# jameschapman19/cca_zoo

Hardware: AMD Instinct MI355X
Metric: CCA fit()/sec at n=1e6 d=4096 k=64 (higher is better)
Workload: dtype f32

## Files before the change

### cca_zoo_amd/csrc/gemm64_big.hip

```cpp
#include <algorithm>
#include <cstdlib>

#include "hip_common.h"

namespace ccz {

typedef double v4f64 __attribute__((ext_vector_type(4)));
typedef double v2f64 __attribute__((ext_vector_type(2)));

constexpr int DT = 128;
constexpr int DK = 16;

constexpr int DS = DT + 2;

constexpr int HM = 64;

template <bool KMAJOR, int W>
struct StagerW {
  static constexpr int NI = W / 32;
  static constexpr int TPR = W / 2;
  static constexpr int RPP = 256 / TPR;
  v2f64 r[NI];
  __device__ __forceinline__ void load(const double* __restrict__ P, int64_t ld, int64_t m0, int64_t mlim, int64_t k0, int tid) {
    if (KMAJOR) {
// ... 22 lines not shown
#pragma unroll
      for (int i = 0; i < NI; ++i) *reinterpret_cast<v2f64*>(dst + (tid / TPR + RPP * i) * stride + 2 * (tid % TPR)) = r[i];
    } else {
      const int kq = tid & 7;
#pragma unroll
      for (int i = 0; i < NI; ++i) {
        const int m = (tid >> 3) + 32 * i;
        dst[(2 * kq) * stride + m] = r[i][0];
        dst[(2 * kq + 1) * stride + m] = r[i][1];
      }
    }
  }
};

template <bool TA, bool TB, int TM>
__global__ __launch_bounds__(256, 2) void k_gemm_f64_pipe(int64_t M, int64_t N, int64_t K, double alpha,
                                                          const double* __restrict__ A, int64_t lda,
                                                          const double* __restrict__ B, int64_t ldb, double beta,
                                                          double* __restrict__ C, int64_t ldc, int lower_only,
                                                          int64_t k_per_split) {
  constexpr int WN = TM == 128 ? 64 : 32;
  constexpr int NB = WN / 16;
  constexpr int SA = TM + 2;
  constexpr int BUF = DK * (SA + DS);
  constexpr int NSTG = TM / 32 + DT / 32;
  extern __shared__ __attribute__((aligned(16))) char smem_p[];
  double* lds = reinterpret_cast<double*>(smem_p);
  const int64_t m0 = int64_t(blockIdx.y) * TM, n0 = int64_t(blockIdx.x) * DT;
  if (lower_only && n0 > m0 + (TM - 1)) return;
  const int tid = threadIdx.x, lane = tid & 63, wave = tid >> 6;
  const int a_off = TM == 128 ? (wave >> 1) * 64 : 0;
  const int b_off = TM == 128 ? (wave & 1) * 64 : wave * 32;

  v4f64 acc[4][NB];
#pragma unroll
  for (int i = 0; i < 4; ++i)
#pragma unroll
    for (int j = 0; j < NB; ++j)
#pragma unroll
      for (int r = 0; r < 4; ++r) acc[i][j][r] = 0.0;

  StagerW<TA, TM> sa;
  StagerW<!TB, DT> sb;
  const bool split = gridDim.z > 1;
  const int64_t kz0 = int64_t(blockIdx.z) * k_per_split;
  const int64_t nkb = (min(K, kz0 + k_per_split) - kz0) / DK;
  if (nkb <= 0) return;

  auto rd = [&](const double* as, int kk, double (&a4)[4], double (&b4)[NB]) {
    const int krow = 4 * kk + (lane >> 4);
    const double* ap = as + krow * SA + a_off + 4 * (lane & 15);
    const v2f64 a01 = *reinterpret_cast<const v2f64*>(ap), a23 = *reinterpret_cast<const v2f64*>(ap + 2);
    a4[0] = a01[0]; a4[1] = a01[1]; a4[2] = a23[0]; a4[3] = a23[1];
    const double* bp = as + DK * SA + krow * DS + b_off + NB * (lane & 15);
    const v2f64 b01 = *reinterpret_cast<const v2f64*>(bp);
    b4[0] = b01[0]; b4[1] = b01[1];
    if constexpr (NB == 4) {
      const v2f64 b23 = *reinterpret_cast<const v2f64*>(bp + 2);
      b4[2] = b23[0]; b4[3] = b23[1];
    }
// ... 83 lines not shown
            v[q + 1] += beta * c01[1];
          }
        }
#pragma unroll
        for (int q = 0; q < NB; q += 2) *reinterpret_cast<v2f64*>(cp + q) = v2f64{v[q], v[q + 1]};
      } else {
#pragma unroll
        for (int tj = 0; tj < NB; ++tj)
          if (nb + tj < N) {
            double v = alpha * acc[ti][tj][r];
            if (beta != 0.0) v += beta * cp[tj];
            cp[tj] = v;
          }
      }
    }
}

bool gemm_f64_big_eligible(bool tA, bool tB, int64_t M, int64_t N, int64_t K, const double* A, int64_t lda,
                           const double* B, int64_t ldb, const double* C, int64_t ldc) {
  (void)tA; (void)tB;
  const int64_t min_tiles = env::once(env::GEMM_BIG_MIN_TILES), min_k = env::once(env::GEMM_BIG_MIN_K);
  if (K % DK != 0 || K < min_k) return false;
  if ((lda | ldb | ldc) & 1) return false;
  if ((reinterpret_cast<uintptr_t>(A) | reinterpret_cast<uintptr_t>(B) | reinterpret_cast<uintptr_t>(C)) & 15) return false;
  if ((M + DT - 1) / DT > 65535) return false;
  const int64_t tiles = (M + DT - 1) / DT * ((N + DT - 1) / DT);
  if (M >= 128 && N >= 128 && tiles >= min_tiles) return true;
  return false;
}

// ... 35 lines not shown
  } while (0)
#define CCZ_LAUNCH_PIPE_T(TM_)                              \
  do {                                                      \
    if (!tA && !tB) CCZ_LAUNCH_PIPE(false, false, TM_);     \
    else if (tA && !tB) CCZ_LAUNCH_PIPE(true, false, TM_);  \
    else if (!tA && tB) CCZ_LAUNCH_PIPE(false, true, TM_);  \
    else CCZ_LAUNCH_PIPE(true, true, TM_);                  \
  } while (0)
  if (use_half) CCZ_LAUNCH_PIPE_T(64);
  else CCZ_LAUNCH_PIPE_T(128);
#undef CCZ_LAUNCH_PIPE_T
#undef CCZ_LAUNCH_PIPE
  CCZ_LAUNCH_CHECK();
}

}
```

### cca_zoo_amd/csrc/gram.hip

```cpp
#include <algorithm>
#include <cstdio>
#include <cstdlib>
#include <cstring>
#include <thread>
#include <vector>

#include "hip_common.h"
#include "gram_map.h"

namespace ccz {

typedef float v16f32 __attribute__((ext_vector_type(16)));
typedef float v4f32 __attribute__((ext_vector_type(4)));
typedef double v4f64 __attribute__((ext_vector_type(4)));
typedef double v2f64 __attribute__((ext_vector_type(2)));

constexpr int BK = 16;

typedef const float __attribute__((address_space(1)))* gptr_f32;
typedef const double __attribute__((address_space(1)))* gptr_f64;

typedef unsigned int v4u32 __attribute__((ext_vector_type(4)));

constexpr int T32 = 256;
// ... 724 lines not shown
  const double sj = (t0 + t1) + (t2 + t3);
  sums[j] = sj;
  pilot[j] = float(sj / double(n));
}

__global__ void k_pilot_from_sums(const double* __restrict__ s, int64_t D, double inv_n, float* __restrict__ pilot) {
  const int64_t j = int64_t(blockIdx.x) * blockDim.x + threadIdx.x;
  if (j < D) pilot[j] = float(s[j] * inv_n);
}

__global__ void k_pilot_fixup(double* __restrict__ G, int64_t D, const double* __restrict__ s_launch, double n,
                              const float* __restrict__ pilot) {
  const int64_t i = blockIdx.y;
  const int64_t j = i + int64_t(blockIdx.x) * blockDim.x + threadIdx.x;
  if (j >= D) return;
  const double pi = double(pilot[i]), pj = double(pilot[j]);
  G[i * D + j] += pi * s_launch[j] + pj * s_launch[i] - n * pi * pj;
}

__global__ __launch_bounds__(256) void k_gram_reduce(const float* __restrict__ partial, const GramTile* __restrict__ tiles, int ntiles,
                                                     int64_t ksplit, double* __restrict__ G, int64_t ldg) {
  const int tile = blockIdx.y;
  const GramTile t = tiles[tile];
  const int e = blockIdx.x * 256 + threadIdx.x;
  const int i = e >> 8, j = e & 255;
  if (i >= t.wa || j >= t.wb) return;
  double acc = 0.0;
  const float* p = partial + int64_t(tile) * (T32 * T32) + e;
  for (int64_t c = 0; c < ksplit; ++c) acc += double(p[c * int64_t(ntiles) * (T32 * T32)]);
  G[(t.out_row + i) * ldg + t.out_col + j] += acc;
}

// ... 276 lines not shown
  hipStream_t st = stream(c);
  constexpr bool is32 = sizeof(T) == 4;
  const int ncu = std::max(1, im->props.multiProcessorCount);
  const int pilot_env = env::once(env::GRAM_PILOT);
  if (pilot_env == 0 || pilot_env == 1) pilot_mode = pilot_env == 1 ? 2 : 0;
  if (!is32) pilot_mode = 0;
  bool split = false;
  if (is32) {
    const char* e = env::once(env::K1_ROUTE);
    const int route_env = !e ? 0 : !strcmp(e, "fp32") ? int(CCZ_K1_FP32) : !strcmp(e, "bf16x2") ? int(CCZ_K1_BF16X2) : 0;
    const int route = c->k1_route != CCZ_K1_AUTO ? c->k1_route : route_env;
    split = (route == CCZ_K1_BF16X2 || (route == CCZ_K1_AUTO && gram_split_worthwhile(n, D))) && n_views <= 16;
    if (split) pilot_mode = 2;
  }
  c->last_route = !is32 ? CCZ_K1_FP64 : (split ? CCZ_K1_BF16X2 : CCZ_K1_FP32);
  if (pilot_mode == 2 && D > 65535) fail(CCZ_EUNSUP, "gram: pilot fix-up supports D <= 65535");
  TileTable tt;
  RowPlan rp;
  if (!split) {
    tt = build_tile_table<T>(c, views, n_views, tile_cache);
    rp = plan_rows<T>(c, views, n_views, n, tt.ntiles, tt.fast);
  }
  const double pilot_thr = env::once(env::GRAM_PILOT_RATIO);
  double* s_launch = s;
  double* sq = nullptr;
  PoolBuf<double> s_own;
  if (pilot_mode != 0) {
    s_own = PoolBuf<double>(c, D * (pilot_mode == 1 ? 2 : 1));
    s_launch = s_own;
    zero(c, s_launch, size_t(D) * 8 * (pilot_mode == 1 ? 2 : 1));
    if (pilot_mode == 1) sq = s_launch + D;
// ... 43 lines not shown
      const double mu = hs[j] / double(n), var = hs[D + j] / double(n) - mu * mu;
      if (!std::isfinite(mu) || !std::isfinite(var)) continue;
      const double sd = var > 0.0 ? std::sqrt(var) : 0.0;
      const double ratio = std::fabs(mu) <= pilot_thr * sd ? 0.0 : (sd > 0.0 ? std::fabs(mu) / sd : 1e300);
      if (ratio > worst) worst = ratio;
    }
    use_pilot = worst > pilot_thr;
    if (use_pilot && D > 65535) fail(CCZ_EUNSUP, "gram: pilot fix-up supports D <= 65535");
  }
  if (use_pilot && !split) {
    pilot = pilot_own = PoolBuf<float>(c, D);
    hipLaunchKernelGGL(k_pilot_from_sums, dim3((unsigned)((D + 255) / 256)), dim3(256), 0, st, s_launch, D, 1.0 / double(n), pilot);
  }

  if (time_it) CCZ_HIP(hipEventRecord(im->ev[0].get(), st));
  if (split) gram_split_f32(c, views, n_views, n, G, D, pilot, s_launch, time_it);
  else if (is32) launch_gram_f32(c, tt, rp, n, G, D, pilot);
  else launch_gram_f64(c, tt, rp, n, G, D);
  CCZ_LAUNCH_CHECK();
  if (time_it) CCZ_HIP(hipEventRecord(im->ev[1].get(), st));
  if (use_pilot) hipLaunchKernelGGL(k_pilot_fixup, dim3((unsigned)((D + 255) / 256), (unsigned)D), dim3(256), 0, st, G, D, s_launch, double(n), pilot);
  if (s_launch != s) hipLaunchKernelGGL(k_vec_add, dim3((unsigned)((D + 255) / 256)), dim3(256), 0, st, s, s_launch, D);
  CCZ_LAUNCH_CHECK();
  if (time_it) {
    CCZ_HIP(hipEventSynchronize(im->ev[1].get()));
    float g = 0.f, cs = 0.f;
    CCZ_HIP(hipEventElapsedTime(&g, im->ev[0].get(), im->ev[1].get()));
    CCZ_HIP(hipEventElapsedTime(&cs, im->ev[2].get(), im->ev[3].get()));
    c->last_gram_ms += g;
    c->last_colsum_ms += cs;
  }
  c->last_pilot = use_pilot ? 1 : 0;
  return use_pilot;
}

bool ensure_pipe(ccz_ctx* c, size_t bytes) {
// ... 289 lines not shown
```

### cca_zoo_amd/csrc/gram_split.hip

```cpp
#include <algorithm>
#include <vector>

#include "hip_common.h"
#include "gram_map.h"
#include "split_mma.h"

namespace ccz {

constexpr int SP_MAXV = 16;

struct SplitPanel {
  int32_t view;
  int32_t col0;
  int32_t width;
  int32_t gcol0;
};

struct SplitViews {
  const float* data[SP_MAXV];
  int64_t ld[SP_MAXV];
};

struct SplitTile {
  int32_t pa, pb;
// ... 156 lines not shown
    if (ti < ti0 || ti >= ti1) continue;
    float* prow = pt + (qr * 128 + ti * 32 + (lane & 31)) * SP_T + qc * 128 + 4 * (lane >> 5);
#pragma unroll
    for (int tj = 0; tj < 4; ++tj) {
      if (sym && tj < ti) continue;
#pragma unroll
      for (int g = 0; g < 4; ++g) {
        const sp_v4f32 v = {acc[ti][tj][4 * g], acc[ti][tj][4 * g + 1], acc[ti][tj][4 * g + 2], acc[ti][tj][4 * g + 3]};
        *reinterpret_cast<sp_v4f32*>(prow + tj * 32 + 8 * g) = v;
      }
    }
  }
}

__global__ __launch_bounds__(256) void k_split_reduce(const float* __restrict__ partial, const SplitTile* __restrict__ tiles, int ntiles,
                                                      int64_t ksplit, double* __restrict__ G, int64_t ldg, const double* __restrict__ msq) {
  const int tile = blockIdx.y;
  const SplitTile t = tiles[tile];
  const int e = (blockIdx.x * 256 + threadIdx.x) * 4;
  const int i = e >> 8, j = e & 255;
  if (i >= t.wa || j >= t.wb) return;
  double a0 = 0.0, a1 = 0.0, a2 = 0.0, a3 = 0.0;
  const float* p = partial + int64_t(tile) * (SP_T * SP_T) + e;
  const int64_t stride = int64_t(ntiles) * (SP_T * SP_T);
  for (int64_t c = 0; c < ksplit; ++c) {
    const sp_v4f32 v = __builtin_nontemporal_load(reinterpret_cast<const sp_v4f32*>(p + c * stride));
    a0 += double(v[0]); a1 += double(v[1]); a2 += double(v[2]); a3 += double(v[3]);
  }
  const double a[4] = {a0, a1, a2, a3};
  double* g = G + (int64_t(t.out_row) + i) * ldg + t.out_col + j;
#pragma unroll
  for (int q = 0; q < 4; ++q) {
    if (j + q >= t.wb) break;
    if (t.diag && j + q < i) continue;
    double v = a[q];
    if (t.diag && i == j + q) v += msq[t.out_row + i];
    g[q] += v;
  }
}

namespace {

std::vector<std::pair<int, int>> split_tile_order(int np) {
  std::vector<std::pair<int, int>> full, dg, rest;
  for (int I = 0; I < np; I += 4)
    for (int J = (I / 8) * 8; J < np; J += 8) {
      std::vector<std::pair<int, int>> blk;
      bool has_diag = false;
      for (int i = I; i < std::min(np, I + 4); ++i)
        for (int j = std::max(i, J); j < std::min(np, J + 8); ++j) { blk.emplace_back(i, j); has_diag = has_diag || i == j; }
      for (const auto& ij : blk) {
        if (blk.size() == 32 && !has_diag) full.push_back(ij);
// ... 177 lines not shown
  CCZ_LAUNCH_CHECK();
  out->tiles = tb.gtiles;
  out->ntiles = tb.ntiles;
  out->ksplit = rp.ksplit;
  c->last_pilot = 1;
  c->last_route = CCZ_K1_BF16X2;
  return true;
}

bool gram_split_worthwhile(int64_t n, int64_t D) {
  const double min_flop = env::live(env::SPLIT_MIN_FLOP);
  return n >= 32768 && D >= 256 && double(n) * double(D) * double(D + 1) >= min_flop;
}

void gram_split_f32(ccz_ctx* c, const ccz_view* views, int n_views, int64_t n, double* G, int64_t D, const float* pilot, double* colsum,
                    bool time_it) {
  Impl* im = impl(c);
  hipStream_t st = stream(c);
  if (n_views > SP_MAXV) fail(CCZ_EUNSUP, "gram (split route): more than %d views", SP_MAXV);
  if (D > 0x7fffffffLL - 256) fail(CCZ_EUNSUP, "gram (split route): stacked width too large");
  int64_t cols[SP_MAXV];
  for (int v = 0; v < n_views; ++v) cols[v] = views[v].cols;
  const SplitTables tb = split_tables(c, cols, n_views);
  SplitViews vws{};
  const bool aligned = split_views_arg(views, n_views, &vws);
  const int np = tb.np, ntiles = tb.ntiles;
  PoolBuf<double> msq(c, D);
  const int ncu = std::max(1, im->props.multiProcessorCount);
  const int64_t max_steps = std::max<int64_t>(1, env::live(env::SPLIT_ROWS) / SP_K);
  const int64_t unit = max_steps * SP_K;
  const double per_row = double(np) * SP_PSTEP / SP_K + double(ntiles) * (SP_T * SP_T * 4) / double(unit);
// ... 25 lines not shown
  hipEvent_t ev[4] = {};
  for (int q = 0; time_it && q < 4; ++q) {
    if (!im->sp_ev[q]) CCZ_HIP(hipEventCreate(im->sp_ev[q].out()));
    ev[q] = im->sp_ev[q].get();
  }
  for (int64_t r0 = 0; r0 < n; r0 += launch_rows) {
    const int64_t rows = std::min(launch_rows, n - r0), ksteps = (rows + SP_K - 1) / SP_K;
    const SplitRowPlan& rp = r0 + launch_rows < n ? rp_full : rp_last;
    zero(c, msq, size_t(D) * 8);
    if (time_it) CCZ_HIP(hipEventRecord(ev[0], st));
    launch_split_pass(c, tb, vws, aligned, r0, rows, ksteps, pilot, planes, msq, colsum);
    if (time_it) CCZ_HIP(hipEventRecord(ev[1], st));
    hipLaunchKernelGGL(k_gram_bf16x2, dim3((unsigned)rp.nblocks), dim3(256), fifo_bytes, st, tb.tiles, ntiles, rp.per_xcd, rp.ksplit, planes.get(), ksteps,
                       rp.steps_per_wg, partial.get());
    if (time_it) CCZ_HIP(hipEventRecord(ev[2], st));
    hipLaunchKernelGGL(k_split_reduce, dim3(64, (unsigned)ntiles), dim3(256), 0, st, partial.get(), tb.tiles, ntiles, rp.ksplit, G, D, msq.get());
    CCZ_LAUNCH_CHECK();
    if (time_it) {
      CCZ_HIP(hipEventRecord(ev[3], st));
      CCZ_HIP(hipEventSynchronize(ev[3]));
      float a = 0.f;
      CCZ_HIP(hipEventElapsedTime(&a, ev[0], ev[1]));
      c->last_split_ms += a;
      CCZ_HIP(hipEventElapsedTime(&a, ev[1], ev[2]));
      c->last_mfma_ms += a;
      CCZ_HIP(hipEventElapsedTime(&a, ev[2], ev[3]));
      c->last_reduce_ms += a;
    }
  }
}

// ... 2 lines not shown
```

### cca_zoo_amd/csrc/hip_common.h

```cpp
#pragma once

#include <hip/hip_runtime.h>

#include <optional>
#include <utility>
#include <vector>

#include "ops.h"

namespace ccz {

template <typename H, auto Destroy>
class Owned {
 public:
  Owned() = default;
  Owned(Owned&& o) noexcept : h_(o.release()) {}
  Owned& operator=(Owned&& o) noexcept { if (this != &o) { reset(); h_ = o.release(); } return *this; }
  Owned(const Owned&) = delete;
  Owned& operator=(const Owned&) = delete;
  ~Owned() { reset(); }
  H get() const { return h_; }
  explicit operator bool() const { return h_ != H(); }
  void reset() { if (h_ != H()) (void)Destroy(h_); h_ = H(); }
  H release() { H h = h_; h_ = H(); return h; }
// ... 155 lines not shown
};

struct GramPartials {
  const GramTile* tiles = nullptr;
  int ntiles = 0;
  int64_t ksplit = 0;
  float* partial = nullptr;
  float* pilot = nullptr;
  double* colsum = nullptr;
  int* tile_plan = nullptr;
  const double* msq = nullptr;
  char* planes = nullptr;
};
bool gram_split_worthwhile(int64_t n, int64_t D);
void gram_split_f32(ccz_ctx* c, const ccz_view* views, int n_views, int64_t n, double* G, int64_t D, const float* pilot, double* colsum,
                    bool time_it);
bool gemm_split_pair_eligible(int64_t M, int64_t N, int64_t K, int64_t K1, int64_t nsplit, const void* A1, int64_t lda1, const void* A2,
                              int64_t lda2, const void* C1, int64_t ldc1, const void* C2, int64_t ldc2);
void gemm_split_pair(ccz_ctx* c, int64_t M, int64_t N, int64_t K, int64_t K1, float alpha, const float* alpha_dev, const float* A1, int64_t lda1,
                     const float* A2, int64_t lda2, const float* gamma32, const double* corr, const double* mean, float* C1,
                     int64_t ldc1, float* C2, int64_t ldc2, int64_t nsplit);
bool project_split_eligible(ccz_ctx* c, int64_t n, int64_t d, int64_t k, int64_t ld, const void* X, int64_t ldo);
void project_split(ccz_ctx* c, const float* X, int64_t n, int64_t d, int64_t ld, const double* mean, const double* W, int64_t k, float* out,
                   int64_t ldo);
bool gram_partials_f32(ccz_ctx* c, const ccz_view* views, int n_views, int64_t n, GramPartials* out);
bool colsum_pilot_f32(ccz_ctx* c, const ccz_view* views, int n_views, int64_t n, int64_t D, double* colsum, float* pilot, double* zero_me,
                      int64_t nzero);
bool gram_partials_split_f32(ccz_ctx* c, const ccz_view* views, int n_views, int64_t n, GramPartials* out);
void gram_partials_release(ccz_ctx* c, GramPartials* gp);

void moments_impl(ccz_ctx* c, int dtype, const ccz_view* views, int n_views, int64_t n_rows,
// ... 11 lines not shown
bool gemm_f32_fifo_split_eligible(int64_t M, int64_t N, int64_t K, int64_t nsplit, const void* C1, int64_t ldc1, const void* C2,
                                  int64_t ldc2);
void gemm_f32_fifo_split(ccz_ctx* c, int64_t M, int64_t N, int64_t K, float alpha, const float* A, int64_t lda, const float* B32,
                         const float* bias32, float* C1, int64_t ldc1, float* C2, int64_t ldc2, int64_t nsplit);

bool gemm_f32_fifo_pair_eligible(int64_t M, int64_t N, int64_t K, int64_t K1, int64_t nsplit, const void* A1, int64_t lda1, const void* A2,
                                 int64_t lda2, const void* C1, int64_t ldc1, const void* C2, int64_t ldc2);
void gemm_f32_fifo_pair(ccz_ctx* c, int64_t M, int64_t N, int64_t K, int64_t K1, float alpha, const float* alpha_dev, const float* A1,
                        int64_t lda1, const float* A2, int64_t lda2, const float* B32, const double* bias64, float* C1, int64_t ldc1,
                        float* C2, int64_t ldc2, int64_t nsplit);

bool gemm_f64_big_eligible(bool tA, bool tB, int64_t M, int64_t N, int64_t K, const double* A, int64_t lda,
                           const double* B, int64_t ldb, const double* C, int64_t ldc);
void gemm_f64_big(ccz_ctx* c, bool tA, bool tB, int64_t M, int64_t N, int64_t K, double alpha, const double* A,
                  int64_t lda, const double* B, int64_t ldb, double beta, double* C, int64_t ldc, bool lower_only);

bool gemm_f64_skinny_eligible(bool tA, bool tB, int64_t M, int64_t N, int64_t K, const double* A, int64_t lda,
                              const double* B, int64_t ldb);
void gemm_f64_skinny(ccz_ctx* c, bool tA, int64_t M, int64_t N, int64_t K, double alpha, const double* A, int64_t lda,
                     const double* B, int64_t ldb, double beta, double* C, int64_t ldc);

void cholinv_batched(ccz_ctx* c, int count, double* const* A, const int64_t* lda, const int64_t* d, double* const* L,
                     const int64_t* ldl, double* const* X, const int64_t* ldx, double* const* T, int* info_dev);
void trinv_batched(ccz_ctx* c, int count, const double* const* L, const int64_t* ldl, const int64_t* d, double* const* X,
                   const int64_t* ldx, const double* const* T);
void copy_lower(ccz_ctx* c, int64_t d, const double* src, int64_t lds_, double* dst, int64_t ldd);
struct MultiGemmArgs {
  const double* A; const double* B; double* C; double* Ct;
  int64_t lda, ldb, ldc, ldct;
  int64_t M, N, K;
// ... 13 lines not shown
```

### cca_zoo_amd/csrc/ops_hip.hip

```cpp
#include <algorithm>
#include <chrono>
#include <string>
#include <vector>
#include <cmath>
#include <cstdio>
#include <cstdlib>
#include <cstring>

#include "hip_common.h"
#include "jacobi_dev.h"
#include "reduce.h"
#include "rng_hash.h"

namespace ccz {

void* dev_alloc(ccz_ctx* c, size_t bytes) {
  Impl* im = impl(c);
  if (bytes == 0) bytes = 8;
  bytes = (bytes + 255) & ~size_t(255);
  int best = -1;
  for (size_t i = 0; i < im->pool.size(); ++i) {
    PoolBlock& b = im->pool[i];
    if (!b.used && b.bytes >= bytes && b.bytes <= bytes + bytes / 4 + 4096) {
      if (best < 0 || b.bytes < im->pool[best].bytes) best = int(i);
// ... 932 lines not shown
  } else {
    for (int64_t bj = nblk - 1; bj >= 0; --bj) {
      const int64_t j = bj * NB;
      const int nb = int(std::min<int64_t>(NB, d - j));
      gemm_ex(c, false, true, r, nb, nb, 1.0, X + j, ldx, invT.get() + bj * NB * NB, NB, 0.0, tmp, NB, X + j, ldx, false);
      if (j > 0)
        gemm(c, false, false, r, j, nb, -1.0, tmp, NB, L + j * ldl, ldl, 1.0, X, ldx);
    }
  }
  };
  if (nblk >= 8) graph_run(c, key, body);
  else body();
}


static const int64_t SB = [] {
  const int64_t v = env::live(env::POTRF_SB);
  return (v == 256 || v == 1024) ? v : int64_t(512);
}();

static void potrf_lower_batched_steps(ccz_ctx* c, int count, double* const* A, const int64_t* d, const int64_t* lda, int* info) {
  for (int b0 = 0; b0 < count; b0 += 8) {
    const int nbt = std::min(8, count - b0);
    std::vector<DBuf> Lb(nbt), Tb(nbt);
    std::vector<double*> Lp(nbt), Tp(nbt);
    std::vector<int64_t> ldl(nbt);
    for (int i = 0; i < nbt; ++i) {
      const int64_t di = d[b0 + i];
      Lb[i] = DBuf(c, di * di);
      Tb[i] = DBuf(c, (di + NB - 1) / NB * NB * NB);
// ... 16 lines not shown
  ccz_ctx* c;
  void* prev;
  StreamSwap(ccz_ctx* c_, hipStream_t s) : c(c_), prev(c_->stream) { c->stream = s; }
  ~StreamSwap() { c->stream = prev; }
};

static void potrf_lower_batched_sb(ccz_ctx* c, int count, double* const* A, const int64_t* d, const int64_t* lda, int* info,
                                   double* const* keep, const TrsmRider* rider = nullptr, int rider_idx = -1) {
  if (count > 8) fail(CCZ_EUNSUP, "potrf_lower_batched_sb: at most 8 matrices per call");
  DBuf rtmp;
  if (rider) rtmp = DBuf(c, rider->r * SB);
  Impl* im = impl(c);
  int64_t dmax = 0;
  for (int i = 0; i < count; ++i) dmax = std::max(dmax, d[i]);
  const int64_t nsb = (dmax + SB - 1) / SB;
  std::vector<DBuf> Ld(count), Xv(count), Tv(count);
  for (int i = 0; i < count; ++i) {
    Ld[i] = DBuf(c, SB * SB);
    Tv[i] = DBuf(c, (SB / NB) * NB * NB);
    if (keep && keep[i]) {
      zero(c, keep[i], size_t((d[i] + SB - 1) / SB) * SB * SB * 8);
    } else {
      Xv[i] = DBuf(c, 2 * SB * SB);
      zero(c, Xv[i], size_t(2) * SB * SB * 8);
    }
  }
  const int nslots = int(nsb) * 8;
  PoolBuf<int> info_dev(c, nslots);
  struct Unwind {
    Impl* im; bool armed = true;
    ~Unwind() { if (armed && im->aux) (void)hipStreamSynchronize(im->aux->st.get()); }
  } unwind{im};

  hipStream_t s_main = stream(c), s_aux = s_main;
  bool la = potrf_lookahead() != 0 && nsb > 1;
  if (la) {
    if (!im->aux && !make_side_stream(im->aux)) la = false;
    if (la) s_aux = im->aux->st.get();
  }
  const hipEvent_t aux_ev[2] = {la ? im->aux->ev[0].get() : nullptr, la ? im->aux->ev[1].get() : nullptr};

  auto factor = [&](int64_t J) {
    const int64_t j0 = J * SB;
    double* Ap[8]; double* Lp[8]; double* Xp[8]; double* Tp[8];
    int64_t la_[8], dd[8], ll[8];
    int cnt = 0;
    bool need_x = false;
    for (int i = 0; i < count; ++i) {
      if (j0 >= d[i]) continue;
      Ap[cnt] = A[i] + j0 * lda[i] + j0;
      la_[cnt] = lda[i];
      dd[cnt] = std::min(SB, d[i] - j0);
      Lp[cnt] = Ld[i].get();
      Xp[cnt] = (keep && keep[i]) ? keep[i] + J * SB * SB : Xv[i].get() + (J & 1) * SB * SB;
      Tp[cnt] = Tv[i].get();
      ll[cnt] = SB;
      need_x = need_x || (keep && keep[i]) || d[i] - j0 - dd[cnt] > 0;
      ++cnt;
    }
    if (cnt > 0) cholinv_batched(c, cnt, Ap, la_, dd, Lp, ll, need_x ? Xp : nullptr, ll, Tp, info_dev + J * 8);
  };

  factor(0);
  for (int64_t J = 0; J < nsb; ++J) {
    const int64_t j0 = J * SB;
    std::vector<DBuf> tmp(count);
    {
      MultiGemmArgs top[8], dg[8];
      int nt = 0;
      for (int i = 0; i < count; ++i) {
        if (j0 >= d[i]) continue;
        const int64_t w = std::min(SB, d[i] - j0), rem = d[i] - j0 - w;
        copy_lower(c, w, Ld[i], SB, A[i] + j0 * lda[i] + j0, lda[i]);
        if (rem <= 0) continue;
        const int64_t w1 = std::min(SB, rem);
        const double* Xj = (keep && keep[i]) ? keep[i] + J * SB * SB : Xv[i].get() + (J & 1) * SB * SB;
        tmp[i] = DBuf(c, rem * w);
        zero(c, tmp[i], size_t(w1) * w * 8);
        MultiGemmArgs& a = top[nt];
        a = MultiGemmArgs{};
        a.A = A[i] + (j0 + w) * lda[i] + j0; a.lda = lda[i]; a.tA = false;
        a.B = Xj; a.ldb = SB; a.tB = true;
        a.C = tmp[i]; a.ldc = w; a.Ct = nullptr; a.ldct = 0;
        a.M = w1; a.N = w; a.K = w; a.alpha = 1.0; a.beta = 1.0; a.lower_only = false; a.ksplit = 4;
        MultiGemmArgs& b = dg[nt];
        b = MultiGemmArgs{};
        b.A = tmp[i]; b.lda = w; b.tA = false;
        b.B = tmp[i]; b.ldb = w; b.tB = true;
        b.C = A[i] + (j0 + w) * lda[i] + (j0 + w); b.ldc = lda[i]; b.Ct = nullptr; b.ldct = 0;
        b.M = w1; b.N = w1; b.K = w; b.alpha = -1.0; b.beta = 1.0; b.lower_only = true; b.ksplit = 4;
        ++nt;
      }
      if (nt > 0) {
        gemm_f64_multi(c, nt, top);
        gemm_f64_multi(c, nt, dg);
      }
    }
    if (J + 1 < nsb) {
      if (la) {
        CCZ_HIP(hipEventRecord(aux_ev[0], s_main));
        CCZ_HIP(hipStreamWaitEvent(s_aux, aux_ev[0], 0));
        {
          StreamSwap sw(c, s_aux);
          const int cap0 = im->chain_cap;
          im->chain_cap = env::once(env::CHAIN_WGS_LA);
          try { factor(J + 1); } catch (...) { im->chain_cap = cap0; throw; }
          im->chain_cap = cap0;
        }
        CCZ_HIP(hipEventRecord(aux_ev[1], s_aux));
      } else {
        factor(J + 1);
      }
    }
    for (int i = 0; i < count; ++i) {
      if (j0 >= d[i]) continue;
      const int64_t w = std::min(SB, d[i] - j0), rem = d[i] - j0 - w;
      if (rem <= 0) continue;
      const int64_t w1 = std::min(SB, rem), rem2 = rem - w1;
      const int64_t j1 = j0 + w;
      copy2d(c, w1, w, tmp[i], w, A[i] + j1 * lda[i] + j0, lda[i]);
      if (rem2 <= 0) continue;
      double* A31 = A[i] + (j1 + w1) * lda[i] + j0;
      double* t2 = tmp[i].get() + w1 * w;
      const double* Xj = (keep && keep[i]) ? keep[i] + J * SB * SB : Xv[i].get() + (J & 1) * SB * SB;
      gemm(c, false, true, rem2, w, w, 1.0, A31, lda[i], Xj, SB, 0.0, t2, w);
      copy2d(c, rem2, w, t2, w, A31, lda[i]);
      gemm(c, false, true, rem2, w1, w, -1.0, t2, w, tmp[i], w, 1.0, A[i] + (j1 + w1) * lda[i] + j1, lda[i]);
      gemm_ex(c, false, true, rem2, rem2, w, -1.0, t2, w, t2, w, 1.0, A[i] + (j1 + w1) * lda[i] + (j1 + w1), lda[i], nullptr, 0, true);
    }
    if (rider && j0 < d[rider_idx]) {
      const int i = rider_idx;
      if (J == 0 && rider->prepare) rider->prepare();
      const int64_t w = std::min(SB, d[i] - j0), rem = d[i] - j0 - w;
      const double* Xinv = keep[i] + J * SB * SB;
      double* X = rider->X;
      gemm(c, false, true, rider->r, w, w, 1.0, X + j0, rider->ldx, Xinv, SB, 0.0, rtmp, SB);
      copy2d(c, rider->r, w, rtmp, SB, X + j0, rider->ldx);
      if (rem > 0)
        gemm(c, false, true, rider->r, rem, w, -1.0, rtmp, SB, A[i] + (j0 + w) * lda[i] + j0, lda[i], 1.0, X + j0 + w, rider->ldx);
    }
    if (la && J + 1 < nsb) CCZ_HIP(hipStreamWaitEvent(s_main, aux_ev[1], 0));
  }
  std::vector<int> got(nslots, 0x7fffffff);
  d2h(c, got.data(), info_dev, size_t(nslots) * sizeof(int));
  unwind.armed = false;
  info_dev.reset();
  for (int i = 0; i < count; ++i) info[i] = 0;
  for (int64_t J = 0; J < nsb; ++J) {
    int cnt = 0;
    for (int i = 0; i < count; ++i) {
      if (J * SB >= d[i]) continue;
      const int v = got[J * 8 + cnt];
      if (v != 0x7fffffff && info[i] == 0) info[i] = int(J * SB) + v;
      ++cnt;
    }
// ... 840 lines not shown
```

Before: 5.820.

## Batch blocked-Cholesky trailing GEMMs and copies; fuse pilot fix-up into split reduce

Restructures the multi-view blocked Cholesky loop. Per-view trailing-update GEMMs (and the rider product) now go into one grouped f64 pipe kernel launch, and the scattered copy/zero operations are deferred into a single batched copy-jobs kernel per block step. Panel and L buffers are double-buffered and persistent, so per-iteration allocations go away. Separately, the pilot-mean fix-up in the split gram route is folded into the split reduce kernel, which drops a separate D×D pass. Risks: ordering of the deferred copies versus the GEMMs that read the panel, and the added lookup cost inside the grouped kernel.

```diff
diff --git a/cca_zoo_amd/csrc/gemm64_big.hip b/cca_zoo_amd/csrc/gemm64_big.hip
--- a/cca_zoo_amd/csrc/gemm64_big.hip
+++ b/cca_zoo_amd/csrc/gemm64_big.hip
@@ -60,11 +60,11 @@
 };
 
 template <bool TA, bool TB, int TM>
-__global__ __launch_bounds__(256, 2) void k_gemm_f64_pipe(int64_t M, int64_t N, int64_t K, double alpha,
-                                                          const double* __restrict__ A, int64_t lda,
-                                                          const double* __restrict__ B, int64_t ldb, double beta,
-                                                          double* __restrict__ C, int64_t ldc, int lower_only,
-                                                          int64_t k_per_split) {
+__device__ __forceinline__ void gemm_f64_pipe_tile(int64_t M, int64_t N, int64_t K, double alpha,
+                                                   const double* __restrict__ A, int64_t lda,
+                                                   const double* __restrict__ B, int64_t ldb, double beta,
+                                                   double* __restrict__ C, int64_t ldc, int lower_only,
+                                                   int64_t k_per_split, int by, int bx, int bz, bool split) {
   constexpr int WN = TM == 128 ? 64 : 32;
   constexpr int NB = WN / 16;
   constexpr int SA = TM + 2;
@@ -72,7 +72,7 @@
   constexpr int NSTG = TM / 32 + DT / 32;
   extern __shared__ __attribute__((aligned(16))) char smem_p[];
   double* lds = reinterpret_cast<double*>(smem_p);
-  const int64_t m0 = int64_t(blockIdx.y) * TM, n0 = int64_t(blockIdx.x) * DT;
+  const int64_t m0 = int64_t(by) * TM, n0 = int64_t(bx) * DT;
   if (lower_only && n0 > m0 + (TM - 1)) return;
   const int tid = threadIdx.x, lane = tid & 63, wave = tid >> 6;
   const int a_off = TM == 128 ? (wave >> 1) * 64 : 0;
@@ -88,8 +88,7 @@
 
   StagerW<TA, TM> sa;
   StagerW<!TB, DT> sb;
-  const bool split = gridDim.z > 1;
-  const int64_t kz0 = int64_t(blockIdx.z) * k_per_split;
+  const int64_t kz0 = int64_t(bz) * k_per_split;
   const int64_t nkb = (min(K, kz0 + k_per_split) - kz0) / DK;
   if (nkb <= 0) return;
 
@@ -203,6 +202,34 @@
           }
       }
     }
+}
+
+template <bool TA, bool TB, int TM>
+__global__ __launch_bounds__(256, 2) void k_gemm_f64_pipe(int64_t M, int64_t N, int64_t K, double alpha,
+                                                          const double* __restrict__ A, int64_t lda,
+                                                          const double* __restrict__ B, int64_t ldb, double beta,
+                                                          double* __restrict__ C, int64_t ldc, int lower_only,
+                                                          int64_t k_per_split) {
+  gemm_f64_pipe_tile<TA, TB, TM>(M, N, K, alpha, A, lda, B, ldb, beta, C, ldc, lower_only, k_per_split, int(blockIdx.y), int(blockIdx.x),
+                                 int(blockIdx.z), gridDim.z > 1);
+}
+
+constexpr int PB_MAX = 8;
+struct PipeBatch {
+  const double* A[PB_MAX];
+  const double* B[PB_MAX];
+  double* C[PB_MAX];
+  int64_t lda[PB_MAX], ldb[PB_MAX], ldc[PB_MAX], M[PB_MAX];
+  int first[PB_MAX + 1];
+  int count;
+};
+
+template <bool TA, bool TB, int TM>
+__global__ __launch_bounds__(256, 2) void k_gemm_f64_pipe_batch(PipeBatch g, int64_t N, int64_t K, double alpha, double beta) {
+  int p = 0;
+  while (p + 1 < g.count && int(blockIdx.y) >= g.first[p + 1]) ++p;
+  gemm_f64_pipe_tile<TA, TB, TM>(g.M[p], N, K, alpha, g.A[p], g.lda[p], g.B[p], g.ldb[p], beta, g.C[p], g.ldc[p], 0, K,
+                                 int(blockIdx.y) - g.first[p], int(blockIdx.x), 0, false);
 }
 
 bool gemm_f64_big_eligible(bool tA, bool tB, int64_t M, int64_t N, int64_t K, const double* A, int64_t lda,
@@ -268,4 +295,41 @@
   CCZ_LAUNCH_CHECK();
 }
 
-}
+bool gemm_f64_nt_batch(ccz_ctx* c, int count, const GemmBatchItem* it, int64_t N, int64_t K, double alpha, double beta) {
+  if (count < 2 || count > PB_MAX || N < 1 || K < DK || K % DK != 0) return false;
+  PipeBatch g{};
+  int64_t tiles128 = 0;
+  const int64_t tn = (N + DT - 1) / DT;
+  for (int i = 0; i < count; ++i) {
+    const GemmBatchItem& a = it[i];
+    if (a.M < 1 || !a.A || !a.B || !a.C) return false;
+    if ((a.lda | a.ldb | a.ldc) & 1) return false;
+    if ((reinterpret_cast<uintptr_t>(a.A) | reinterpret_cast<uintptr_t>(a.B) | reinterpret_cast<uintptr_t>(a.C)) & 15) return false;
+    tiles128 += (a.M + DT - 1) / DT * tn;
+  }
+  const int ncu = std::max(1, impl(c)->props.multiProcessorCount);
+  const int tm_rows = tiles128 < int64_t(ncu) ? HM : DT;
+  int64_t total = 0;
+  for (int i = 0; i < count; ++i) {
+    const GemmBatchItem& a = it[i];
+    g.A[i] = a.A; g.B[i] = a.B; g.C[i] = a.C; g.lda[i] = a.lda; g.ldb[i] = a.ldb; g.ldc[i] = a.ldc; g.M[i] = a.M;
+    g.first[i] = int(total);
+    total += (a.M + tm_rows - 1) / tm_rows;
+  }
+  if (total > 65535) return false;
+  g.first[count] = int(total);
+  g.count = count;
+  const size_t lds_p = size_t(2) * DK * (tm_rows + 2 + DS) * 8;
+  const dim3 grid((unsigned)tn, (unsigned)total, 1);
+  if (tm_rows == HM) {
+    CCZ_HIP(hipFuncSetAttribute(reinterpret_cast<const void*>(&k_gemm_f64_pipe_batch<false, true, HM>), hipFuncAttributeMaxDynamicSharedMemorySize, int(lds_p)));
+    hipLaunchKernelGGL((k_gemm_f64_pipe_batch<false, true, HM>), grid, dim3(256), lds_p, stream(c), g, N, K, alpha, beta);
+  } else {
+    CCZ_HIP(hipFuncSetAttribute(reinterpret_cast<const void*>(&k_gemm_f64_pipe_batch<false, true, DT>), hipFuncAttributeMaxDynamicSharedMemorySize, int(lds_p)));
+    hipLaunchKernelGGL((k_gemm_f64_pipe_batch<false, true, DT>), grid, dim3(256), lds_p, stream(c), g, N, K, alpha, beta);
+  }
+  CCZ_LAUNCH_CHECK();
+  return true;
+}
+
+}
diff --git a/cca_zoo_amd/csrc/gram.hip b/cca_zoo_amd/csrc/gram.hip
--- a/cca_zoo_amd/csrc/gram.hip
+++ b/cca_zoo_amd/csrc/gram.hip
@@ -762,8 +762,7 @@
   const int64_t i = blockIdx.y;
   const int64_t j = i + int64_t(blockIdx.x) * blockDim.x + threadIdx.x;
   if (j >= D) return;
-  const double pi = double(pilot[i]), pj = double(pilot[j]);
-  G[i * D + j] += pi * s_launch[j] + pj * s_launch[i] - n * pi * pj;
+  G[i * D + j] += pilot_fixup_term(double(pilot[i]), double(pilot[j]), s_launch[i], s_launch[j], n);
 }
 
 __global__ __launch_bounds__(256) void k_gram_reduce(const float* __restrict__ partial, const GramTile* __restrict__ tiles, int ntiles,
@@ -1070,7 +1069,7 @@
     if (split) pilot_mode = 2;
   }
   c->last_route = !is32 ? CCZ_K1_FP64 : (split ? CCZ_K1_BF16X2 : CCZ_K1_FP32);
-  if (pilot_mode == 2 && D > 65535) fail(CCZ_EUNSUP, "gram: pilot fix-up supports D <= 65535");
+  if (pilot_mode == 2 && !split && D > 65535) fail(CCZ_EUNSUP, "gram: pilot fix-up supports D <= 65535");
   TileTable tt;
   RowPlan rp;
   if (!split) {
@@ -1144,12 +1143,12 @@
   }
 
   if (time_it) CCZ_HIP(hipEventRecord(im->ev[0].get(), st));
-  if (split) gram_split_f32(c, views, n_views, n, G, D, pilot, s_launch, time_it);
+  if (split) gram_split_f32(c, views, n_views, n, G, D, pilot, s_launch, time_it, true);
   else if (is32) launch_gram_f32(c, tt, rp, n, G, D, pilot);
   else launch_gram_f64(c, tt, rp, n, G, D);
   CCZ_LAUNCH_CHECK();
   if (time_it) CCZ_HIP(hipEventRecord(im->ev[1].get(), st));
-  if (use_pilot) hipLaunchKernelGGL(k_pilot_fixup, dim3((unsigned)((D + 255) / 256), (unsigned)D), dim3(256), 0, st, G, D, s_launch, double(n), pilot);
+  if (use_pilot && !split) hipLaunchKernelGGL(k_pilot_fixup, dim3((unsigned)((D + 255) / 256), (unsigned)D), dim3(256), 0, st, G, D, s_launch, double(n), pilot);
   if (s_launch != s) hipLaunchKernelGGL(k_vec_add, dim3((unsigned)((D + 255) / 256)), dim3(256), 0, st, s, s_launch, D);
   CCZ_LAUNCH_CHECK();
   if (time_it) {
diff --git a/cca_zoo_amd/csrc/gram_split.hip b/cca_zoo_amd/csrc/gram_split.hip
--- a/cca_zoo_amd/csrc/gram_split.hip
+++ b/cca_zoo_amd/csrc/gram_split.hip
@@ -194,7 +194,8 @@
 }
 
 __global__ __launch_bounds__(256) void k_split_reduce(const float* __restrict__ partial, const SplitTile* __restrict__ tiles, int ntiles,
-                                                      int64_t ksplit, double* __restrict__ G, int64_t ldg, const double* __restrict__ msq) {
+                                                      int64_t ksplit, double* __restrict__ G, int64_t ldg, const double* __restrict__ msq,
+                                                      const float* __restrict__ pilot, const double* __restrict__ s_launch, double n) {
   const int tile = blockIdx.y;
   const SplitTile t = tiles[tile];
   const int e = (blockIdx.x * 256 + threadIdx.x) * 4;
@@ -208,14 +209,19 @@
     a0 += double(v[0]); a1 += double(v[1]); a2 += double(v[2]); a3 += double(v[3]);
   }
   const double a[4] = {a0, a1, a2, a3};
-  double* g = G + (int64_t(t.out_row) + i) * ldg + t.out_col + j;
+  const int64_t gi = int64_t(t.out_row) + i, gj = int64_t(t.out_col) + j;
+  double* g = G + gi * ldg + gj;
+  double pi = 0.0, si = 0.0;
+  if (pilot) { pi = double(pilot[gi]); si = s_launch[gi]; }
 #pragma unroll
   for (int q = 0; q < 4; ++q) {
     if (j + q >= t.wb) break;
     if (t.diag && j + q < i) continue;
     double v = a[q];
     if (t.diag && i == j + q) v += msq[t.out_row + i];
-    g[q] += v;
+    double out = g[q] + v;
+    if (pilot) out += pilot_fixup_term(pi, double(pilot[gj + q]), si, s_launch[gj + q], n);
+    g[q] = out;
   }
 }
 
@@ -423,7 +429,8 @@
 }
 
 void gram_split_f32(ccz_ctx* c, const ccz_view* views, int n_views, int64_t n, double* G, int64_t D, const float* pilot, double* colsum,
-                    bool time_it) {
+                    bool time_it, bool fixup) {
+  if (fixup && (!pilot || !colsum)) fail(CCZ_EINVAL, "gram (split route): the fused pilot fix-up needs the pilot and the column sums");
   Impl* im = impl(c);
   hipStream_t st = stream(c);
   if (n_views > SP_MAXV) fail(CCZ_EUNSUP, "gram (split route): more than %d views", SP_MAXV);
@@ -479,7 +486,9 @@
     hipLaunchKernelGGL(k_gram_bf16x2, dim3((unsigned)rp.nblocks), dim3(256), fifo_bytes, st, tb.tiles, ntiles, rp.per_xcd, rp.ksplit, planes.get(), ksteps,
                        rp.steps_per_wg, partial.get());
     if (time_it) CCZ_HIP(hipEventRecord(ev[2], st));
-    hipLaunchKernelGGL(k_split_reduce, dim3(64, (unsigned)ntiles), dim3(256), 0, st, partial.get(), tb.tiles, ntiles, rp.ksplit, G, D, msq.get());
+    const bool fix = fixup && r0 + launch_rows >= n;
+    hipLaunchKernelGGL(k_split_reduce, dim3(64, (unsigned)ntiles), dim3(256), 0, st, partial.get(), tb.tiles, ntiles, rp.ksplit, G, D, msq.get(),
+                       fix ? pilot : static_cast<const float*>(nullptr), fix ? colsum : static_cast<const double*>(nullptr), double(n));
     CCZ_LAUNCH_CHECK();
     if (time_it) {
       CCZ_HIP(hipEventRecord(ev[3], st));
diff --git a/cca_zoo_amd/csrc/hip_common.h b/cca_zoo_amd/csrc/hip_common.h
--- a/cca_zoo_amd/csrc/hip_common.h
+++ b/cca_zoo_amd/csrc/hip_common.h
@@ -193,7 +193,10 @@
 };
 bool gram_split_worthwhile(int64_t n, int64_t D);
 void gram_split_f32(ccz_ctx* c, const ccz_view* views, int n_views, int64_t n, double* G, int64_t D, const float* pilot, double* colsum,
-                    bool time_it);
+                    bool time_it, bool fixup);
+__device__ __forceinline__ double pilot_fixup_term(double pi, double pj, double si, double sj, double n) {
+  return pi * sj + pj * si - n * pi * pj;
+}
 bool gemm_split_pair_eligible(int64_t M, int64_t N, int64_t K, int64_t K1, int64_t nsplit, const void* A1, int64_t lda1, const void* A2,
                               int64_t lda2, const void* C1, int64_t ldc1, const void* C2, int64_t ldc2);
 void gemm_split_pair(ccz_ctx* c, int64_t M, int64_t N, int64_t K, int64_t K1, float alpha, const float* alpha_dev, const float* A1, int64_t lda1,
@@ -235,6 +238,14 @@
                            const double* B, int64_t ldb, const double* C, int64_t ldc);
 void gemm_f64_big(ccz_ctx* c, bool tA, bool tB, int64_t M, int64_t N, int64_t K, double alpha, const double* A,
                   int64_t lda, const double* B, int64_t ldb, double beta, double* C, int64_t ldc, bool lower_only);
+
+struct GemmBatchItem {
+  const double* A; int64_t lda;
+  const double* B; int64_t ldb;
+  double* C; int64_t ldc;
+  int64_t M;
+};
+bool gemm_f64_nt_batch(ccz_ctx* c, int count, const GemmBatchItem* items, int64_t N, int64_t K, double alpha, double beta);
 
 bool gemm_f64_skinny_eligible(bool tA, bool tB, int64_t M, int64_t N, int64_t K, const double* A, int64_t lda,
                               const double* B, int64_t ldb);
diff --git a/cca_zoo_amd/csrc/ops_hip.hip b/cca_zoo_amd/csrc/ops_hip.hip
--- a/cca_zoo_amd/csrc/ops_hip.hip
+++ b/cca_zoo_amd/csrc/ops_hip.hip
@@ -970,6 +970,61 @@
 }
 
 
+constexpr int CJ_MAX = 32, CJ_ROWS = 8;
+struct CopyJob {
+  const double* src; double* dst;
+  int64_t lds_, ldd, rows, cols;
+  bool lower;
+};
+struct CopyJobsArg {
+  const double* src[CJ_MAX];
+  double* dst[CJ_MAX];
+  int64_t lds_[CJ_MAX], ldd[CJ_MAX];
+  int rows[CJ_MAX], cols[CJ_MAX], lower[CJ_MAX];
+  int first[CJ_MAX + 1];
+  int count;
+};
+
+__global__ __launch_bounds__(256) void k_copy_jobs(CopyJobsArg g) {
+  int p = 0;
+  while (p + 1 < g.count && int(blockIdx.x) >= g.first[p + 1]) ++p;
+  const int r0 = (int(blockIdx.x) - g.first[p]) * CJ_ROWS;
+  const int rows = min(CJ_ROWS, g.rows[p] - r0), cols = g.cols[p];
+  const double* __restrict__ src = g.src[p];
+  double* __restrict__ dst = g.dst[p];
+  const int64_t ls = g.lds_[p], ld = g.ldd[p];
+  const bool lower = g.lower[p] != 0;
+  for (int e = threadIdx.x; e < rows * cols; e += 256) {
+    const int r = r0 + e / cols, cc = e % cols;
+    if (lower && cc > r) continue;
+    dst[int64_t(r) * ld + cc] = src ? src[int64_t(r) * ls + cc] : 0.0;
+  }
+}
+
+static void copy_jobs(ccz_ctx* c, const std::vector<CopyJob>& jobs) {
+  CopyJobsArg g{};
+  int total = 0;
+  auto launch = [&] {
+    if (g.count == 0) return;
+    g.first[g.count] = total;
+    hipLaunchKernelGGL(k_copy_jobs, dim3((unsigned)total), dim3(256), 0, stream(c), g);
+    CCZ_LAUNCH_CHECK();
+    g = CopyJobsArg{};
+    total = 0;
+  };
+  for (const CopyJob& j : jobs) {
+    if (j.rows <= 0 || j.cols <= 0) continue;
+    if (!j.dst || j.rows > 0x7fffffff / CJ_ROWS || j.cols > 0x7fffffff / CJ_ROWS) fail(CCZ_EINVAL, "copy_jobs: bad job");
+    const int i = g.count++;
+    g.src[i] = j.src; g.dst[i] = j.dst; g.lds_[i] = j.lds_; g.ldd[i] = j.ldd;
+    g.rows[i] = int(j.rows); g.cols[i] = int(j.cols); g.lower[i] = j.lower ? 1 : 0;
+    g.first[i] = total;
+    total += int((j.rows + CJ_ROWS - 1) / CJ_ROWS);
+    if (g.count == CJ_MAX) launch();
+  }
+  launch();
+}
+
 static const int64_t SB = [] {
   const int64_t v = env::live(env::POTRF_SB);
   return (v == 256 || v == 1024) ? v : int64_t(512);
@@ -1016,17 +1071,23 @@
   int64_t dmax = 0;
   for (int i = 0; i < count; ++i) dmax = std::max(dmax, d[i]);
   const int64_t nsb = (dmax + SB - 1) / SB;
-  std::vector<DBuf> Ld(count), Xv(count), Tv(count);
+  std::vector<DBuf> Ld(count), Xv(count), Tv(count), Pn(count);
+  std::vector<int64_t> pn_half(count);
+  std::vector<CopyJob> jobs;
   for (int i = 0; i < count; ++i) {
-    Ld[i] = DBuf(c, SB * SB);
+    Ld[i] = DBuf(c, 2 * SB * SB);
     Tv[i] = DBuf(c, (SB / NB) * NB * NB);
+    pn_half[i] = std::max<int64_t>(0, d[i] - SB) * SB;
+    Pn[i] = DBuf(c, 2 * pn_half[i]);
+    jobs.push_back(CopyJob{nullptr, Pn[i].get(), 0, SB, std::min(SB, d[i] - SB), SB, false});
     if (keep && keep[i]) {
-      zero(c, keep[i], size_t((d[i] + SB - 1) / SB) * SB * SB * 8);
+      jobs.push_back(CopyJob{nullptr, keep[i], 0, SB, (d[i] + SB - 1) / SB * SB, SB, false});
     } else {
       Xv[i] = DBuf(c, 2 * SB * SB);
-      zero(c, Xv[i], size_t(2) * SB * SB * 8);
-    }
-  }
+      jobs.push_back(CopyJob{nullptr, Xv[i].get(), 0, SB, 2 * SB, SB, false});
+    }
+  }
+  copy_jobs(c, jobs);
   const int nslots = int(nsb) * 8;
   PoolBuf<int> info_dev(c, nslots);
   struct Unwind {
@@ -1053,7 +1114,7 @@
       Ap[cnt] = A[i] + j0 * lda[i] + j0;
       la_[cnt] = lda[i];
       dd[cnt] = std::min(SB, d[i] - j0);
-      Lp[cnt] = Ld[i].get();
+      Lp[cnt] = Ld[i].get() + (J & 1) * SB * SB;
       Xp[cnt] = (keep && keep[i]) ? keep[i] + J * SB * SB : Xv[i].get() + (J & 1) * SB * SB;
       Tp[cnt] = Tv[i].get();
       ll[cnt] = SB;
@@ -1066,29 +1127,29 @@
   factor(0);
   for (int64_t J = 0; J < nsb; ++J) {
     const int64_t j0 = J * SB;
-    std::vector<DBuf> tmp(count);
+    jobs.clear();
+    auto panel = [&](int i) { return Pn[i].get() + (J & 1) * pn_half[i]; };
     {
       MultiGemmArgs top[8], dg[8];
       int nt = 0;
       for (int i = 0; i < count; ++i) {
         if (j0 >= d[i]) continue;
         const int64_t w = std::min(SB, d[i] - j0), rem = d[i] - j0 - w;
-        copy_lower(c, w, Ld[i], SB, A[i] + j0 * lda[i] + j0, lda[i]);
+        jobs.push_back(CopyJob{Ld[i].get() + (J & 1) * SB * SB, A[i] + j0 * lda[i] + j0, SB, lda[i], w, w, true});
         if (rem <= 0) continue;
         const int64_t w1 = std::min(SB, rem);
         const double* Xj = (keep && keep[i]) ? keep[i] + J * SB * SB : Xv[i].get() + (J & 1) * SB * SB;
-        tmp[i] = DBuf(c, rem * w);
-        zero(c, tmp[i], size_t(w1) * w * 8);
+        double* pn = panel(i);
         MultiGemmArgs& a = top[nt];
         a = MultiGemmArgs{};
         a.A = A[i] + (j0 + w) * lda[i] + j0; a.lda = lda[i]; a.tA = false;
         a.B = Xj; a.ldb = SB; a.tB = true;
-        a.C = tmp[i]; a.ldc = w; a.Ct = nullptr; a.ldct = 0;
+        a.C = pn; a.ldc = w; a.Ct = nullptr; a.ldct = 0;
         a.M = w1; a.N = w; a.K = w; a.alpha = 1.0; a.beta = 1.0; a.lower_only = false; a.ksplit = 4;
         MultiGemmArgs& b = dg[nt];
         b = MultiGemmArgs{};
-        b.A = tmp[i]; b.lda = w; b.tA = false;
-        b.B = tmp[i]; b.ldb = w; b.tB = true;
+        b.A = pn; b.lda = w; b.tA = false;
+        b.B = pn; b.ldb = w; b.tB = true;
         b.C = A[i] + (j0 + w) * lda[i] + (j0 + w); b.ldc = lda[i]; b.Ct = nullptr; b.ldct = 0;
         b.M = w1; b.N = w1; b.K = w; b.alpha = -1.0; b.beta = 1.0; b.lower_only = true; b.ksplit = 4;
         ++nt;
@@ -1114,33 +1175,51 @@
         factor(J + 1);
       }
     }
+    const bool ride = rider && j0 < d[rider_idx];
+    if (ride && J == 0 && rider->prepare) rider->prepare();
+    const int64_t rw = ride ? std::min(SB, d[rider_idx] - j0) : 0;
+    GemmBatchItem rest[9], colj[8];
+    int nr = 0, nc = 0;
     for (int i = 0; i < count; ++i) {
       if (j0 >= d[i]) continue;
       const int64_t w = std::min(SB, d[i] - j0), rem = d[i] - j0 - w;
       if (rem <= 0) continue;
       const int64_t w1 = std::min(SB, rem), rem2 = rem - w1;
       const int64_t j1 = j0 + w;
-      copy2d(c, w1, w, tmp[i], w, A[i] + j1 * lda[i] + j0, lda[i]);
+      double* pn = panel(i);
+      jobs.push_back(CopyJob{pn, A[i] + j1 * lda[i] + j0, w, lda[i], rem, w, false});
+      if (rem2 > 0) jobs.push_back(CopyJob{nullptr, Pn[i].get() + ((J + 1) & 1) * pn_half[i], 0, SB, std::min(SB, rem2), SB, false});
       if (rem2 <= 0) continue;
-      double* A31 = A[i] + (j1 + w1) * lda[i] + j0;
-      double* t2 = tmp[i].get() + w1 * w;
+      double* t2 = pn + w1 * w;
       const double* Xj = (keep && keep[i]) ? keep[i] + J * SB * SB : Xv[i].get() + (J & 1) * SB * SB;
-      gemm(c, false, true, rem2, w, w, 1.0, A31, lda[i], Xj, SB, 0.0, t2, w);
-      copy2d(c, rem2, w, t2, w, A31, lda[i]);
-      gemm(c, false, true, rem2, w1, w, -1.0, t2, w, tmp[i], w, 1.0, A[i] + (j1 + w1) * lda[i] + j1, lda[i]);
-      gemm_ex(c, false, true, rem2, rem2, w, -1.0, t2, w, t2, w, 1.0, A[i] + (j1 + w1) * lda[i] + (j1 + w1), lda[i], nullptr, 0, true);
-    }
-    if (rider && j0 < d[rider_idx]) {
+      rest[nr++] = GemmBatchItem{A[i] + (j1 + w1) * lda[i] + j0, lda[i], Xj, SB, t2, w, rem2};
+      colj[nc++] = GemmBatchItem{t2, w, pn, w, A[i] + (j1 + w1) * lda[i] + j1, lda[i], rem2};
+    }
+    bool rider_product_done = false;
+    if (ride && rw == SB && nr > 0) {
+      rest[nr] = GemmBatchItem{rider->X + j0, rider->ldx, keep[rider_idx] + J * SB * SB, SB, rtmp.get(), SB, rider->r};
+      rider_product_done = gemm_f64_nt_batch(c, nr + 1, rest, SB, SB, 1.0, 0.0);
+    }
+    if (!rider_product_done && !gemm_f64_nt_batch(c, nr, rest, SB, SB, 1.0, 0.0))
+      for (int t = 0; t < nr; ++t) gemm(c, false, true, rest[t].M, SB, SB, 1.0, rest[t].A, rest[t].lda, rest[t].B, rest[t].ldb, 0.0, rest[t].C, rest[t].ldc);
+    if (!gemm_f64_nt_batch(c, nc, colj, SB, SB, -1.0, 1.0))
+      for (int t = 0; t < nc; ++t) gemm(c, false, true, colj[t].M, SB, SB, -1.0, colj[t].A, colj[t].lda, colj[t].B, colj[t].ldb, 1.0, colj[t].C, colj[t].ldc);
+    for (int t = 0; t < nr; ++t) {
+      const double* t2 = rest[t].C;
+      double* Arest = colj[t].C + SB;
+      gemm_ex(c, false, true, rest[t].M, rest[t].M, SB, -1.0, t2, SB, t2, SB, 1.0, Arest, colj[t].ldc, nullptr, 0, true);
+    }
+    if (ride) {
       const int i = rider_idx;
-      if (J == 0 && rider->prepare) rider->prepare();
-      const int64_t w = std::min(SB, d[i] - j0), rem = d[i] - j0 - w;
+      const int64_t w = rw, rem = d[i] - j0 - w;
       const double* Xinv = keep[i] + J * SB * SB;
       double* X = rider->X;
-      gemm(c, false, true, rider->r, w, w, 1.0, X + j0, rider->ldx, Xinv, SB, 0.0, rtmp, SB);
-      copy2d(c, rider->r, w, rtmp, SB, X + j0, rider->ldx);
+      if (!rider_product_done) gemm(c, false, true, rider->r, w, w, 1.0, X + j0, rider->ldx, Xinv, SB, 0.0, rtmp, SB);
+      jobs.push_back(CopyJob{rtmp.get(), X + j0, SB, rider->ldx, rider->r, w, false});
       if (rem > 0)
-        gemm(c, false, true, rider->r, rem, w, -1.0, rtmp, SB, A[i] + (j0 + w) * lda[i] + j0, lda[i], 1.0, X + j0 + w, rider->ldx);
-    }
+        gemm(c, false, true, rider->r, rem, w, -1.0, rtmp, SB, panel(i), w, 1.0, X + j0 + w, rider->ldx);
+    }
+    copy_jobs(c, jobs);
     if (la && J + 1 < nsb) CCZ_HIP(hipStreamWaitEvent(s_main, aux_ev[1], 0));
   }
   std::vector<int> got(nslots, 0x7fffffff);
```

Result: no change. 5.799 (-0.4%).
